# usnistgov/optbayesexpt

Hardware: AMD Instinct MI355X
Metric: model-evals/sec (settings x particles) per opt_setting+update cycle, fp64 (higher is better)
Workload: dtype f64; 1 GPU; c3: Lorentzian 3-param, 65 536 settings x 1 048 576 particles; n_settings=65536, n_particles=1048576, settings_per_rank=65536

## Files before the change

include/obe_hip.h:

```cpp
#ifndef OBE_HIP_H
#define OBE_HIP_H

#include <stdint.h>

#ifdef __cplusplus
extern "C" {
#endif

#define OBE_API __attribute__((visibility("default")))

#define OBE_ABI_VERSION 3
#define OBE_MAX_CONSTS 8
#define OBE_MAX_CHANNELS 8
#define OBE_MAX_SETDIMS 8
#define OBE_MAX_DIMS 32
#define OBE_FAST_DIMS 16
#define OBE_CLOUD_MAX_DIMS 1024

enum obe_model_id {
    OBE_MODEL_LORENTZ = 1,
    OBE_MODEL_LINE_AB = 2,
    OBE_MODEL_LINE_MB = 3,
    OBE_MODEL_FIRST_PARAM = 4,
    OBE_MODEL_RABI = 5,
// ... 173 lines not shown
                        void* d_ws, int64_t ws_bytes, void* stream);

#define OBE_WS_RESULT_OFFSET 2
#define OBE_WS_RESULT_TAIL(d_ws, ws_bytes) ((double*)((char*)(d_ws) + ((ws_bytes) & ~(int64_t)7) - 48))
#define OBE_NOISE_FROM_MOMENTS(r0, r1, r2, r3) \
    (-(int64_t)1 - ((int64_t)(r0) | ((int64_t)(r1) << 5) | ((int64_t)(r2) << 10) | ((int64_t)(r3) << 15)))
#define OBE_SWEEP_SHIFTED 1
#define OBE_SWEEP_SAFE 2
#define OBE_SWEEP_SPECULATIVE 8
#define OBE_SWEEP_NOWAIT 16
#define OBE_SWEEP_CELLS 4
#define OBE_CELL_RHO_INV 4
#define OBE_CELL_ORDER 28
#define OBE_CELL_MAX 128
#define OBE_CELL_MIN_GAIN 2
OBE_API int obe_sweep_cells_plan(double x_min, double x_max, double d, int64_t n_settings, int64_t n_draws);
#define OBE_SWEEP_BINS 32
#define OBE_BIN_MAX 128
OBE_API int obe_sweep_bins_plan(double x_min, double x_max, double d, int64_t n_settings, int64_t n_draws);
OBE_API int obe_sweep_bins_eval_waves(int64_t n_settings);
OBE_API int obe_sweep_settings_per_lane(int64_t n_settings);
OBE_API int obe_sweep_settings_per_lane_for(int64_t n_settings, int64_t n_draws);
OBE_API int obe_sweep_utility(const obe_model* m,
                      const double* d_settings, int64_t ld_s, int64_t n_settings,
                      const double* d_particles, int64_t ld_p, int64_t n_particles,
                      const double* d_weights, const int64_t* d_draw_idx, int64_t n_draws,
                      const double* d_moments, int32_t shifted,
                      const double* d_noise_var, int64_t noise_ld,
                      const double* d_cost, double cost_scalar,
                      double* d_yvar, double* d_utility,
                      double* h_best, int64_t* h_best_idx, double* h_kappa,
                      void* d_ws, int64_t ws_bytes, void* stream);
OBE_API int64_t obe_sweep_bins_keep_bytes(int64_t n_draws);
#define OBE_SWEEP_BINS_KEPT 64
OBE_API int obe_sweep_utility_keep(const obe_model* m,
                      const double* d_settings, int64_t ld_s, int64_t n_settings,
                      const double* d_particles, int64_t ld_p, int64_t n_particles,
                      const double* d_weights, const int64_t* d_draw_idx, int64_t n_draws,
                      const double* d_moments, int32_t shifted,
                      const double* d_noise_var, int64_t noise_ld,
                      const double* d_cost, double cost_scalar,
                      double* d_yvar, double* d_utility,
                      double* h_value, int64_t* h_index, double* h_factor,
                      void* d_ws, int64_t ws_bytes, void* stream,
                      void* d_keep, int64_t keep_bytes);

OBE_API int obe_yspace_variance(const double* d_yspace, int64_t n_draws, int32_t n_channels,
                        int64_t n_settings, double* d_yvar, void* stream);
OBE_API int obe_utility_argmax(const double* d_yvar, int32_t n_channels, int64_t n_settings,
                       const double* d_noise_var, int64_t noise_ld,
                       const double* d_cost, double cost_scalar,
                       double* d_utility, double* h_best, int64_t* h_best_idx,
                       void* d_ws, int64_t ws_bytes, void* stream);
OBE_API int obe_argmax(const double* d_v, int64_t n, double* h_best, int64_t* h_best_idx,
               void* d_ws, int64_t ws_bytes, void* stream);

OBE_API int obe_eval_draws(const obe_model* m, const double* d_settings, int64_t ld_s, int64_t n_settings,
                   const double* d_particles, int64_t ld_p, int64_t n_particles,
                   const int64_t* d_draw_idx, int64_t n_draws, double* d_yspace, void* stream);
OBE_API int obe_yspace_add_noise(double* d_yspace, int64_t n_draws, int32_t n_channels, int64_t n_settings,
                         const double* d_noise, void* stream);
OBE_API int obe_yspace_maxmin(const double* d_yspace, int64_t n_draws, int64_t n_columns, double* d_span2, void* stream);
OBE_API int obe_yspace_entropy(const double* d_yspace, int64_t n_draws, int64_t n_columns, int32_t as_variance,
                       double* d_scratch, double* d_out, void* stream);
OBE_API int obe_kld_utility(const double* d_entropy_y, int32_t n_channels, int64_t n_settings,
                    const double* d_entropy_noise, double* d_utility, void* stream);
// ... 127 lines not shown
```

optbayesexpt_amd/_lib.py:

```python
import ctypes
import os
import re

import numpy as np

HERE = os.path.dirname(os.path.abspath(__file__))
LIB_PATH = os.path.join(HERE, "lib", "libobe_hip.so")
HEADER_PATH = os.path.join(os.path.dirname(HERE), "include", "obe_hip.h")



def _header_constants(path=HEADER_PATH):
    text = open(path).read()
    return {k: int(v) for k, v in re.findall(r"^#define\s+(OBE_[A-Z_]+)\s+(-?\d+)\s*(?:/\*.*)?$", text, flags=re.M)}


_H = _header_constants()
OBE_ABI_VERSION = _H["OBE_ABI_VERSION"]
OBE_MAX_CONSTS = _H["OBE_MAX_CONSTS"]
OBE_MAX_CHANNELS = _H["OBE_MAX_CHANNELS"]
OBE_MAX_SETDIMS = _H["OBE_MAX_SETDIMS"]
OBE_MAX_DIMS = _H["OBE_MAX_DIMS"]
OBE_FAST_DIMS = _H["OBE_FAST_DIMS"]
OBE_CLOUD_MAX_DIMS = _H["OBE_CLOUD_MAX_DIMS"]
# ... 53 lines not shown
def _ctype(c_type):
    m = re.fullmatch(r"(?:const\s+)?(\w+)\s*(\**)", c_type)
    if m and m[2]:
        return _POINTERS.get(m[1] + m[2], c_void_p)
    if m and m[1] in _SCALARS:
        return _SCALARS[m[1]]
    raise TypeError(f"no ctypes binding for the C type {c_type!r} of include/obe_hip.h")


def _prototypes(header_path=HEADER_PATH):
    text = re.sub(r"/\*.*?\*/", "", open(header_path).read(), flags=re.S)
    protos = {}
    for ret, name, params in re.findall(r"^OBE_API\s+([^(]+?)\s*\b(obe_\w+)\s*\(([^)]*)\)\s*;", text, flags=re.M):
        args = []
        for param in [] if params.strip() == "void" else params.split(","):
            m = re.fullmatch(r"(.+?)\s*\b(\w+)", param.strip())
            if m is None:
                raise TypeError(f"{name}: cannot read the parameter {param.strip()!r} of include/obe_hip.h")
            args.append((_ctype(m[1]), m[2]))
        protos[name] = (_ctype(ret), args)
    return protos


PROTOTYPES = _prototypes()


MODEL_ENTRY_POINTS = ("obe_model_validate", "obe_workspace_bytes", "obe_sweep_settings_per_lane",
                      "obe_sweep_settings_per_lane_for", "obe_bayes_update_model",
                      "obe_bayes_update_model_moments", "obe_bayes_update_model_moments_enqueue",
                      "obe_strict_sums",
                      "obe_bayes_update_sweep",
                      "obe_eval_over_particles",
                      "obe_eval_over_settings", "obe_sweep_utility", "obe_sweep_kernel_time", "obe_sweep_timing",
                      "obe_sweep_utility_keep", "obe_sweep_bins_keep_bytes",
                      "obe_eval_draws",
                      "obe_predictive_workspace_bytes", "obe_predictive_moments", "obe_predictive_quantiles",
                      "obe_predictive_score_workspace_bytes", "obe_predictive_logpdf", "obe_predictive_tails",
                      "obe_predictive_reading_workspace_bytes", "obe_predictive_reading_quantiles",
                      "obe_output_covariance_workspace_bytes", "obe_output_covariance",
                      "obe_records_loglik_workspace_bytes", "obe_records_loglik",
                      "obe_output_cross_covariance_workspace_bytes", "obe_output_cross_covariance",
                      "obe_signal_noise_likelihood", "obe_signal_noise_workspace_bytes", "obe_signal_noise_variance")


class HipLib:

    def __init__(self, path=LIB_PATH, plugin=False, allow_variant=False):
        if not os.path.exists(path):
            raise ImportError(
                f"{path} not found: the HIP library has not been built.  Run "
                "`python -m optbayesexpt_amd.build` (needs hipcc).  optbayesexpt_amd has "
                "no CPU fallback.")
        import torch
        self.path = path
        self.cdll = ctypes.CDLL(path, mode=ctypes.RTLD_LOCAL if plugin else ctypes.RTLD_GLOBAL)
        names = MODEL_ENTRY_POINTS + ("obe_abi_version", "obe_last_error", "obe_source_fingerprint") if plugin \
            else tuple(PROTOTYPES)
        for name in names:
            restype, params = PROTOTYPES[name]
            fn = getattr(self.cdll, name)
            fn.restype = restype
            fn.argtypes = [ctype for ctype, _ in params]
        abi = self.cdll.obe_abi_version()
        if abi != OBE_ABI_VERSION:
            raise ImportError(f"libobe_hip ABI {abi} does not match this package ({OBE_ABI_VERSION})")
        from . import build
        built_from = self.cdll.obe_source_fingerprint().decode()
# ... 170 lines not shown
```

optbayesexpt_amd/csrc/obe_sweep.hip:

```cpp
#include <cstdlib>

#include "obe_update.h"
#include "obe_sweep_common.h"
#include "obe_sweep_cells.h"
#include "obe_sweep_bins.h"

namespace obe {

constexpr int kMaxChunks = 1024;
constexpr int kFinMaxBlocks = 65536;

static int64_t argmax_slots(int64_t n_settings) {
    return std::max<int64_t>(kMaxBlocks, (n_settings + kFinSettings - 1) / kFinSettings);
}

static SweepPlan plan_sweep(int64_t ns, int64_t nd, int cost = 1, int max_spt = 8) {
    SweepPlan p;
    p.spt = ns >= 4096 || (ns >= 2048 && nd >= 131072) ? 8 : (ns >= 1024 ? 4 : (ns >= 512 ? 2 : 1));
    if (p.spt > max_spt) p.spt = max_spt;
    p.tiles_x = static_cast<int>((ns + (int64_t)kWave * p.spt - 1) / ((int64_t)kWave * p.spt));
    const int64_t by_work = static_cast<int64_t>((double)ns * (double)nd * (double)cost / 1.25e6);
    const int64_t target_blocks = std::max<int64_t>(1536, std::min<int64_t>(4608, by_work));
    int64_t want = (target_blocks + p.tiles_x - 1) / p.tiles_x;
    if (want > 8) want = (want + 7) / 8 * 8;
// ... 665 lines not shown
    double replaced = (double)n_settings * (double)n_draws * kDirectSlots;
    if (cells == 3) {
        const double ncells = std::floor((x_max / d - x_min / d) * (1.0 / LorentzCells::kWidth)) + 1.0;
        replaced = (double)n_draws * std::ceil(ncells / kWave) * kWave * kCellSlots;
    }
    const double bins = (double)n_settings * OBE_BIN_MAX * kBinEvalSlots + (double)n_draws * kBinDrawSlots + kBinFixedSlots;
    return replaced >= OBE_CELL_MIN_GAIN * bins ? 3 : 1;
}

int obe_sweep_bins_eval_waves(int64_t n_settings) { return plan_bin_eval_waves(n_settings < 1 ? 1 : n_settings); }

int obe_sweep_settings_per_lane_for(int64_t n_settings, int64_t n_draws) {
    if (n_settings < 1) n_settings = 1;
    if (n_draws < 1) return obe_sweep_settings_per_lane(n_settings);
    if (one_workgroup_sweep(n_settings, n_draws)) return 1;
    return plan_sweep(n_settings, n_draws).spt;
}

int64_t obe_workspace_bytes(int64_t n_particles, int64_t n_settings, int32_t n_channels, int32_t n_dims) {
    if (n_particles < 1) n_particles = 1;
    if (n_settings < 1) n_settings = 1;
    if (n_channels < 1) n_channels = 1;
    if (n_dims < 1) n_dims = 1;
    const int packed_w = max_packed_width(n_dims);
    int64_t b = sweep_ws_bytes_bound(n_settings, n_particles, n_channels, packed_w);
    b = std::max(b, moments_ws_bytes(n_dims));
    b = std::max(b, update_ws_bytes(n_dims));
    b = std::max(b, scan_ws_bytes(n_particles));
    b = std::max(b, resample_wide_ws_bytes(n_dims));
    return b + 64 * (int64_t)sizeof(double);
}

int64_t obe_sweep_bins_keep_bytes(int64_t n_draws) { return BinKeepLayout::bytes(n_draws < 1 ? 1 : n_draws); }

int obe_sweep_utility(const obe_model* m, const double* d_settings, int64_t ld_s, int64_t n_settings,
                      const double* d_particles, int64_t ld_p, int64_t n_particles, const double* d_weights,
                      const int64_t* d_draw_idx, int64_t n_draws, const double* d_moments, int32_t shifted,
                      const double* d_noise_var, int64_t noise_ld, const double* d_cost, double cost_scalar,
                      double* d_yvar, double* d_utility, double* h_best, int64_t* h_best_idx, double* h_kappa,
                      void* d_ws, int64_t ws_bytes, void* stream) {
    return obe_sweep_utility_keep(m, d_settings, ld_s, n_settings, d_particles, ld_p, n_particles, d_weights, d_draw_idx,
                                  n_draws, d_moments, shifted, d_noise_var, noise_ld, d_cost, cost_scalar, d_yvar, d_utility,
                                  h_best, h_best_idx, h_kappa, d_ws, ws_bytes, stream, nullptr, 0);
}

int obe_sweep_utility_keep(const obe_model* m, const double* d_settings, int64_t ld_s, int64_t n_settings,
                           const double* d_particles, int64_t ld_p, int64_t n_particles, const double* d_weights,
                           const int64_t* d_draw_idx, int64_t n_draws, const double* d_moments, int32_t shifted,
                           const double* d_noise_var, int64_t noise_ld, const double* d_cost, double cost_scalar,
                           double* d_yvar, double* d_utility, double* h_best, int64_t* h_best_idx, double* h_kappa,
                           void* d_ws, int64_t ws_bytes, void* stream, void* d_keep, int64_t keep_bytes) {
    if (!d_noise_var || !d_yvar || !d_utility) return bad_arg("obe_sweep_utility: bad output/noise pointer");
    if (d_keep && reinterpret_cast<uintptr_t>(d_keep) % 16) return bad_arg("obe_sweep_utility_keep: d_keep is not 16-byte aligned");
    SweepCall c;
    if (int rc = prepare_sweep(SweepInputs{m, d_settings, ld_s, n_settings, d_particles, ld_p, n_particles, d_weights,
                                           d_draw_idx, n_draws, d_moments, shifted, d_ws, ws_bytes, d_keep, keep_bytes}, c))
        return rc;
    const obe_model& mm = c.mm;
    SweepPlan& plan = c.plan;
    SweepArgs& a = c.a;
    const SweepWs& w = c.w;
    hipStream_t st = as_stream(stream);
    UtilArgs ua;
    if (int rc = make_util_args(ua, d_noise_var, noise_ld, d_cost, cost_scalar, mm.n_channels, mm.n_params)) return rc;
    const bool speculative = shifted & OBE_SWEEP_SPECULATIVE;
    const bool nowait = speculative || (shifted & OBE_SWEEP_NOWAIT);
// ... 202 lines not shown
```

optbayesexpt_amd/csrc/obe_sweep_bins.h:

```cpp
#pragma once
#include "obe_sweep_common.h"

namespace obe {

struct BinPlan {
    double origin;
    int nbins;
    unsigned poison;
};
constexpr int kBinMinmaxBlocks = 256;
constexpr int kBinMaxUnits = 2048;
constexpr int kBinChunk = 1024;
constexpr int kBinFoldGroups = 16;
constexpr int kBinScanPer = kBinMaxUnits / kBlock;
constexpr double kBinEvalSlots = 8.0 * LorentzBins::kOrder + 16.0;
constexpr double kBinDrawSlots = 4.0 * LorentzBins::kOrder + 8.0;
constexpr double kBinFixedSlots = 80.0 * 3.9e7;

struct BinUnits {
    int nunits;
    int64_t per;
};
static BinUnits plan_bin_units(int64_t nd) {
    BinUnits u;
// ... 2 lines not shown
    u.nunits = static_cast<int>((nd + u.per - 1) / u.per);
    return u;
}
struct BinEvalShape {
    int waves, groups;
};
constexpr BinEvalShape kBinEvalShapes[] = {{8, 1}, {6, 2}, {3, 4}};
constexpr int kBinEvalWavesPerCU = 12, kChipCUs = 256;
static int plan_bin_eval_waves(int64_t ns) {
    const int64_t groups = (ns + kWave - 1) / kWave;
    for (const BinEvalShape& f : kBinEvalShapes)
        if (groups <= (int64_t)kChipCUs * f.groups * (kBinEvalWavesPerCU / (f.groups * f.waves))) return f.waves;
    return 1;
}
static int64_t bin_max_items(int64_t nd) { return (nd + kBinChunk - 1) / kBinChunk + LorentzBins::kMaxBins; }
struct BinLayout {
    static constexpr int64_t kPlan = 0, kRan = 3, kStarts = 4;
    static constexpr int64_t kMinmax = kStarts + 132;
    static constexpr int64_t kTotals = kMinmax + 3 * kBinMinmaxBlocks;
    static constexpr int64_t kCounts = kTotals + LorentzBins::kMaxBins / 2;
    static constexpr int64_t kCoef = kCounts + (int64_t)LorentzBins::kMaxBins * kBinMaxUnits / 2;
    static constexpr int64_t kPart = kCoef + (int64_t)LorentzBins::kMaxBins * LorentzBins::kRow;
    static int64_t sorted(int64_t nd) { return kPart + bin_max_items(nd) * LorentzBins::kRow; }
    static int64_t doubles(int64_t nd) { return sorted(nd) + 4 * nd; }
};
static_assert(BinLayout::kPart % 2 == 0 && LorentzBins::kRow % 2 == 0, "the sorted records are 16-byte aligned");

struct BinKeep {
    BinPlan plan;
    unsigned mark;
    int nd;
    unsigned long long dbits;
    unsigned mismatch;
    unsigned pad[7];
};
static_assert(sizeof(BinKeep) == 64, "the head of the keep buffer is 16 ints");
constexpr unsigned kBinKeepMark = 0x6b455042u;
struct BinKeepLayout {
    static constexpr int64_t kStarts = sizeof(BinKeep) / sizeof(int);
    static constexpr int64_t kDest = (kStarts + 2 * (LorentzBins::kMaxBins + 2) + 3) & ~(int64_t)3;
    static int64_t bytes(int64_t nd) { return ((kDest + nd) * (int64_t)sizeof(int) + 15) & ~(int64_t)15; }
};

#ifndef OBE_PLUGIN_MODEL_HEADER
struct BinSweepPtrs {
    BinPlan* plan;
    unsigned* ran;
    int* binstart;
    int* itemstart;
    BinKeep* keep;
    int* dest;
    int* code;
    int reuse;
    int keep_nd;
    unsigned long long keep_dbits;
    unsigned call;
    double* minmax;
    int* totals;
    int* counts;
    double* coef;
    double* part;
    double* sorted;
};

__device__ __forceinline__ bool bin_keep_refused(const BinSweepPtrs& q) {
    if (!q.reuse) return false;
    const BinKeep* k = q.keep;
    return !(k->mark == kBinKeepMark && k->nd == q.keep_nd && k->dbits == q.keep_dbits);
}

__device__ __forceinline__ double bin_tau0(const SweepArgs& a, int64_t p) {
    double w;
    const int64_t src = draw_source(a, p, w);
    return a.particles[src] / a.m.consts[0];
}

__device__ __forceinline__ void bin_record(const SweepArgs& a, int64_t p, double2& ra, double2& rb) {
    using M = Lorentz<1>;
    static_assert(packed_width<M>() == 4 && M::NPK == 3, "the sorted records are 32 bytes");
    double w, pk[4];
    const int64_t src = draw_source(a, p, w);
    const double sw = sqrt(w);
    M::pack(ParamRef{a.particles + src, a.ld_p}, a.moments + 2, a.m, sw, pk);
    ra = double2{pk[0], pk[1]};
    rb = double2{pk[2], sw};
}

constexpr int kBinRankBits = 24;
static_assert((((int64_t)1 << 30) + kBinMaxUnits - 1) / kBinMaxUnits <= ((int64_t)1 << kBinRankBits)
                  && LorentzBins::kMaxBins <= (1 << (31 - kBinRankBits)),
              "a unit of a cloud of 2^30 draws (BinForm::selected) has at most 2^19 draws: rank and bin share an int");
__device__ __forceinline__ int bin_code(int bin, int rank) { return (bin << kBinRankBits) | rank; }

__global__ __launch_bounds__(kBlock) void bin_minmax_kernel(SweepArgs a, BinSweepPtrs q) {
    constexpr int NW = kBlock / kWave;
    __shared__ double slo[NW], shi[NW];
    __shared__ int sbad[NW];
    if (sweep_aborted(a.abort)) return;
    if (q.keep && blockIdx.x == 0 && threadIdx.x == 0) q.keep->mark = 0u;
    double* __restrict__ minmax = q.minmax;
    double lo = INFINITY, hi = -INFINITY;
    int bad = 0;
    for (int64_t p = (int64_t)blockIdx.x * kBlock + threadIdx.x; p < a.nd; p += (int64_t)gridDim.x * kBlock) {
        const double t = bin_tau0(a, p);
        bad |= !(fabs(t) <= kDblMax);
        lo = fmin(lo, t);
        hi = fmax(hi, t);
    }
#pragma unroll
    for (int o = kWave / 2; o > 0; o >>= 1) {
        lo = fmin(lo, __shfl_down(lo, o, kWave));
        hi = fmax(hi, __shfl_down(hi, o, kWave));
        bad |= __shfl_down(bad, o, kWave);
    }
    if ((threadIdx.x & (kWave - 1)) == 0) {
        slo[threadIdx.x / kWave] = lo;
        shi[threadIdx.x / kWave] = hi;
        sbad[threadIdx.x / kWave] = bad;
    }
    __syncthreads();
    if (threadIdx.x != 0) return;
    for (int g = 1; g < NW; ++g) {
        lo = fmin(lo, slo[g]);
        hi = fmax(hi, shi[g]);
        bad |= sbad[g];
    }
    minmax[blockIdx.x] = lo;
    minmax[kBinMinmaxBlocks + blockIdx.x] = hi;
    minmax[2 * kBinMinmaxBlocks + blockIdx.x] = bad ? 1.0 : 0.0;
}

__device__ __forceinline__ BinPlan bin_plan_of(const SweepArgs& a, const double* __restrict__ minmax, int nblocks) {
// ... 3 lines not shown
#pragma unroll
    for (int g = 0; g < kBinMinmaxBlocks / kWave; ++g) {
        const int b = g * kWave + lane;
        const bool have = b < nblocks;
        lo = fmin(lo, have ? minmax[b] : INFINITY);
        hi = fmax(hi, have ? minmax[kBinMinmaxBlocks + b] : -INFINITY);
        bad |= have ? minmax[2 * kBinMinmaxBlocks + b] != 0.0 : 0;
    }
#pragma unroll
    for (int o = kWave / 2; o > 0; o >>= 1) {
        lo = fmin(lo, __shfl_xor(lo, o, kWave));
        hi = fmax(hi, __shfl_xor(hi, o, kWave));
        bad |= __shfl_xor(bad, o, kWave);
    }
    const double d = a.m.consts[0];
    const double n = floor((hi - lo) * (1.0 / LorentzBins::kWidth)) + 1.0;
    const bool ok = !bad && d > 0.0 && d <= kDblMax && fabs(lo) <= kDblMax && fabs(hi) <= kDblMax
                    && n <= (double)LorentzBins::kMaxBins;
    return BinPlan{lo, ok ? static_cast<int>(n) : 0, ok ? 0u : 1u};
}

__device__ __forceinline__ int wave_exclusive(int v, int& total) {
    const int lane = threadIdx.x & (kWave - 1);
    int inc = v;
#pragma unroll
    for (int o = 1; o < kWave; o <<= 1) {
        const int up = __shfl_up(inc, o, kWave);
        inc += lane >= o ? up : 0;
    }
    total = __shfl(inc, kWave - 1, kWave);
    return inc - v;
}

template <bool SCATTER>
__global__ __launch_bounds__(kBlock) void bin_group_kernel(SweepArgs a, int64_t per, int nunits, int mm_blocks,
                                                           BinSweepPtrs q) {
    using LB = LorentzBins;
    if (sweep_aborted(a.abort)) return;
    const int lane = threadIdx.x & (kWave - 1);
    const int unit = blockIdx.x * (kBlock / kWave) + threadIdx.x / kWave;
    BinPlan plan;
    if constexpr (SCATTER) {
        plan = *q.plan;
        if (q.keep && blockIdx.x == 0 && threadIdx.x == 0) {
            q.keep->nd = static_cast<int>(a.nd);
            q.keep->dbits = q.keep_dbits;
            q.keep->mismatch = 0u;
            q.keep->mark = kBinKeepMark;
        }
    } else {
        plan = bin_plan_of(a, q.minmax, mm_blocks);
        if (blockIdx.x == 0 && threadIdx.x == 0) *q.plan = plan;
    }
    const int nbins = __builtin_amdgcn_readfirstlane(plan.nbins);
    if (nbins == 0) return;
    int c0 = 0, c1 = 0;
    if constexpr (SCATTER) {
        const int t0 = q.totals[lane], t1 = q.totals[lane + kWave];
        int sum0, sum1, isum0, isum1;
        const int e0 = wave_exclusive(t0, sum0), e1 = sum0 + wave_exclusive(t1, sum1);
        const int i0 = wave_exclusive((t0 + kBinChunk - 1) / kBinChunk, isum0);
        const int i1 = isum0 + wave_exclusive((t1 + kBinChunk - 1) / kBinChunk, isum1);
        if (unit == 0) {
            q.binstart[lane] = e0;
            q.binstart[lane + kWave] = e1;
            q.itemstart[lane] = i0;
            q.itemstart[lane + kWave] = i1;
            if (lane == 0) {
                q.binstart[LB::kMaxBins] = sum0 + sum1;
                q.itemstart[LB::kMaxBins] = isum0 + isum1;
            }
        }
        if (unit >= nunits) return;
        c0 = e0 + q.counts[lane * kBinMaxUnits + unit];
        c1 = e1 + q.counts[(lane + kWave) * kBinMaxUnits + unit];
    }
    if (unit >= nunits) return;
    const int64_t begin = (int64_t)unit * per;
    const int64_t end = begin + per < a.nd ? begin + per : a.nd;
    for (int64_t i0 = begin; i0 < end; i0 += kWave) {
        const int64_t i = i0 + lane;
        const bool live = i < end;
        if constexpr (SCATTER) {
            const int code = live ? q.code[i] : 0;
            const int bin = code >> kBinRankBits;
            const int first0 = __shfl(c0, bin & (kWave - 1), kWave), first1 = __shfl(c1, bin & (kWave - 1), kWave);
            const int pos = (bin < kWave ? first0 : first1) + (code & ((1 << kBinRankBits) - 1));
            if (live && pos >= 0 && pos < a.nd) {
                double2 ra, rb;
                bin_record(a, i, ra, rb);
                double2* __restrict__ out = reinterpret_cast<double2*>(q.sorted) + 2 * (int64_t)pos;
                out[0] = ra;
                out[1] = rb;
            }
            if (q.dest && live) q.dest[i] = pos;
        } else {
            const int bin = live ? LB::bin_of(plan.origin, bin_tau0(a, i), nbins) : -1;
            int rank = 0;
            unsigned long long todo = __ballot(live);
            while (todo) {
                const int b = __builtin_amdgcn_readlane(bin, __builtin_ctzll(todo));
                const unsigned long long same = __ballot(bin == b);
                const int figure = __builtin_amdgcn_readlane(b < kWave ? c0 : c1, b & (kWave - 1));
                if (bin == b) rank = figure + __popcll(same & ((1ull << lane) - 1ull));
                const int n = __popcll(same);
                if (lane == (b & (kWave - 1))) {
                    if (b < kWave) c0 += n;
                    else c1 += n;
                }
                todo &= ~same;
            }
            if (live) q.code[i] = bin_code(bin, rank);
        }
    }
    if constexpr (!SCATTER) {
        q.counts[lane * kBinMaxUnits + unit] = c0;
        q.counts[(lane + kWave) * kBinMaxUnits + unit] = c1;
    }
}

__global__ __launch_bounds__(kBlock) void bin_scatter_pack_kernel(SweepArgs a, BinSweepPtrs q) {
    using LB = LorentzBins;
    if (sweep_aborted(a.abort)) return;
    if (bin_keep_refused(q)) return;
    const int nbins = __builtin_amdgcn_readfirstlane(q.plan->nbins);
    if (nbins <= 0 || nbins > LB::kMaxBins) return;
    const double origin = q.plan->origin;
    for (int64_t p = (int64_t)blockIdx.x * kBlock + threadIdx.x; p < a.nd; p += (int64_t)gridDim.x * kBlock) {
        double2 ra, rb;
        bin_record(a, p, ra, rb);
        const int pos = q.dest[p];
        const double t = (ra.x - origin) * (1.0 / LB::kWidth);
        bool ok = t >= 0.0 && t < (double)nbins && pos >= 0 && pos < a.nd;
        if (ok) {
            const int b = LB::bin_of(origin, ra.x, nbins);
            ok = q.binstart[b] <= pos && pos < q.binstart[b + 1];
        }
        if (ok) {
            double2* __restrict__ out = reinterpret_cast<double2*>(q.sorted) + 2 * (int64_t)pos;
            out[0] = ra;
            out[1] = rb;
        } else {
            q.keep->mismatch = q.call;
        }
    }
}

__global__ __launch_bounds__(kBlock) void bin_scan_kernel(int nunits, BinSweepPtrs q, const unsigned* abort) {
    __shared__ int wsum[kBlock / kWave];
    if (sweep_aborted(abort)) return;
    const int nbins = __builtin_amdgcn_readfirstlane(q.plan->nbins);
    const int bin = blockIdx.x;
    if (nbins == 0) return;
    if (bin >= nbins) {
        if (threadIdx.x == 0) q.totals[bin] = 0;
        return;
    }
    int* __restrict__ row = q.counts + bin * kBinMaxUnits;
    int v[kBinScanPer], mine = 0;
#pragma unroll
    for (int u = 0; u < kBinScanPer; ++u) {
        const int k = threadIdx.x * kBinScanPer + u;
        v[u] = k < nunits ? row[k] : 0;
        mine += v[u];
    }
    int wtotal;
    int before = wave_exclusive(mine, wtotal);
    if ((threadIdx.x & (kWave - 1)) == 0) wsum[threadIdx.x / kWave] = wtotal;
    __syncthreads();
    int total = 0;
#pragma unroll
    for (int g = 0; g < kBlock / kWave; ++g) {
        if (g < (int)threadIdx.x / kWave) before += wsum[g];
        total += wsum[g];
    }
#pragma unroll
    for (int u = 0; u < kBinScanPer; ++u) {
// ... 9 lines not shown
    constexpr int H = (N + 1) / 2;
    const bool upper = (lane & DIST) != 0;
    double k[H];
#pragma unroll
    for (int i = 0; i < H; ++i) {
        const double lo = v[i], hi = H + i < N ? v[H + i] : 0.0;
        const double mine = upper ? hi : lo, send = upper ? lo : hi;
        k[i] = mine + __shfl_xor(send, DIST, kWave);
    }
    if constexpr (DIST > 1) {
        halving_reduce<H, DIST / 2>(k, lane, out);
    } else {
        static_assert(H == 2, "64 lanes x 2 values: at most 128 sums");
        out[0] = k[0];
        out[1] = k[1];
    }
}
template <int N>
__device__ __forceinline__ int halving_index(int lane, int e) {
    int n[7];
    n[0] = N;
#pragma unroll
    for (int l = 0; l < 6; ++l) n[l + 1] = (n[l] + 1) / 2;
    int j = e;
    bool real = true;
#pragma unroll
    for (int l = 5; l >= 0; --l) {
        j += ((lane >> (5 - l)) & 1) * n[l + 1];
        real = real && j < n[l];
    }
    return real ? j : -1;
}

__global__ __launch_bounds__(kWave) void bin_moments_kernel(BinSweepPtrs q, const unsigned* abort) {
    using LB = LorentzBins;
    if (sweep_aborted(abort)) return;
    if (bin_keep_refused(q)) return;
    const int nbins = __builtin_amdgcn_readfirstlane(q.plan->nbins);
    if (nbins == 0) return;
    const int lane = threadIdx.x, item = blockIdx.x;
    if (item >= q.itemstart[LB::kMaxBins]) return;
    const int s0 = q.itemstart[lane], s1 = q.itemstart[lane + kWave];
    const int bin = __popcll(__ballot(lane < nbins && s0 <= item)) + __popcll(__ballot(lane + kWave < nbins && s1 <= item)) - 1;
    const int first = q.binstart[bin] + (item - q.itemstart[bin]) * kBinChunk;
    const int last = q.binstart[bin + 1];
    const int end = first + kBinChunk < last ? first + kBinChunk : last;
    const double tb = LB::centre(q.plan->origin, bin);
    const double2* __restrict__ rec = reinterpret_cast<const double2*>(q.sorted);
    LB::Sums z;
    z.clear();
    int i = first + lane;
    double2 ra = double2{0.0, 0.0}, rb = ra;
    if (i < end) {
        ra = rec[2 * (int64_t)i];
        rb = rec[2 * (int64_t)i + 1];
    }
    while (i < end) {
        const int in = i + kWave;
        double2 na = ra, nb = rb;
        if (in < end) {
            na = rec[2 * (int64_t)in];
            nb = rec[2 * (int64_t)in + 1];
        }
        const double pk[4] = {ra.x, ra.y, rb.x, rb.y};
        LB::add_draw(tb, pk, z);
        ra = na;
        rb = nb;
        i = in;
    }
    double v[LB::kCoefs], kept[2];
#pragma unroll
    for (int k = 0; k < LB::kOrder; ++k) {
        v[k] = z.M1[k];
        v[LB::kOrder + k] = z.M2[k];
        v[2 * LB::kOrder + k] = z.M3[k];
    }
    v[3 * LB::kOrder] = z.c1;
    v[3 * LB::kOrder + 1] = z.c2;
    halving_reduce<LB::kCoefs, kWave / 2>(v, lane, kept);
    double* __restrict__ out = q.part + (int64_t)item * LB::kRow;
#pragma unroll
    for (int e = 0; e < 2; ++e) {
        const int j = halving_index<LB::kCoefs>(lane, e);
        if (j < 0) continue;
        const bool m3 = j >= 2 * LB::kOrder && j < 3 * LB::kOrder;
        out[j] = kept[e] * (m3 ? (double)(j - 2 * LB::kOrder + 1) : 1.0);
    }
}

__global__ __launch_bounds__(kBinFoldGroups * kWave) void bin_fold_kernel(BinSweepPtrs q, const unsigned* abort) {
    using LB = LorentzBins;
    __shared__ double acc[kBinFoldGroups][kWave];
    if (sweep_aborted(abort)) return;
    if (bin_keep_refused(q)) return;
    const int nbins = __builtin_amdgcn_readfirstlane(q.plan->nbins);
    const int bin = blockIdx.x >> 1, co = (blockIdx.x & 1) * kWave + (threadIdx.x & (kWave - 1));
    if (bin >= nbins) return;
    const int first = __builtin_amdgcn_readfirstlane(q.itemstart[bin]);
    const int n = __builtin_amdgcn_readfirstlane(q.itemstart[bin + 1]) - first;
    if (n == 0) return;
    const bool live = co < LB::kCoefs;
// ... 122 lines not shown
        S2 = a2 + C2;
    }
    if (blockIdx.x == 0 && threadIdx.x == 0) *q.ran = seq;
    if (W > 1 && wid != 0) return;
    if (!f.yvar) {
        if (s >= a.ns) return;
        a.part1[s] = S1;
        a.part2[s] = S2;
        a.cs_out[s] = 0.0;
        return;
    }
    const int64_t group = (int64_t)blockIdx.x * G + grp;
    if (group * kWave >= a.ns) return;
    double kappa = 0.0;
    Best best{-INFINITY, INT64_MAX};
    if (s < a.ns) {
        const double var = variance_of_moments(0.0 + S1, 0.0 + S2, f.full_mode ? a.moments[0] : 1.0, 0.0, kappa);
        f.yvar[s] = var;
        const double u = utility_of(&var, 1, 1, s, f.ua);
        f.utility[s] = u;
        best = Best{u, s};
    }
    wave_best(best, kappa);
    if (lane == 0) {
        f.bv[group] = best.v;
        f.bi[group] = best.i;
        f.bk[group] = kappa;
    }
}

struct BinForm {
    bool on = false;
    BinSweepPtrs q{};

    static bool selected(const obe_model& m, int flags, int64_t ns, const int64_t* d_draw_idx, int64_t n_draws,
                         int64_t nd) {
        return (flags & OBE_SWEEP_BINS) && nd <= ((int64_t)1 << 30) && expansion_applies(m, flags, ns, d_draw_idx, n_draws);
    }
    void carve(double* base, double* packed, int64_t nd, const obe_model& m, int flags, const int64_t* d_draw_idx,
               void* d_keep, int64_t keep_bytes) {
        using BL = BinLayout;
        q.plan = reinterpret_cast<BinPlan*>(base + BL::kPlan);
        q.ran = reinterpret_cast<unsigned*>(base + BL::kRan);
        q.binstart = reinterpret_cast<int*>(base + BL::kStarts);
        q.itemstart = q.binstart + LorentzBins::kMaxBins + 2;
        q.minmax = base + BL::kMinmax;
        q.totals = reinterpret_cast<int*>(base + BL::kTotals);
        q.counts = reinterpret_cast<int*>(base + BL::kCounts);
        q.coef = base + BL::kCoef;
        q.part = base + BL::kPart;
        q.sorted = base + BL::sorted(nd);
        q.code = reinterpret_cast<int*>(packed);
        if (d_keep && !d_draw_idx && keep_bytes >= BinKeepLayout::bytes(nd)) {
            static std::atomic<unsigned> calls{0};
            int* ints = static_cast<int*>(d_keep);
            q.keep = static_cast<BinKeep*>(d_keep);
            q.plan = &q.keep->plan;
            q.binstart = ints + BinKeepLayout::kStarts;
            q.itemstart = q.binstart + LorentzBins::kMaxBins + 2;
            q.dest = ints + BinKeepLayout::kDest;
            q.code = q.dest;
            q.reuse = (flags & OBE_SWEEP_BINS_KEPT) != 0;
            q.keep_nd = static_cast<int>(nd);
            memcpy(&q.keep_dbits, &m.consts[0], sizeof q.keep_dbits);
            q.call = ++calls;
            if (q.call == 0u) q.call = ++calls;
        }
    }
    int before(const SweepArgs& a, hipStream_t st) const {
        if (!q.reuse) return 0;
        bin_scatter_pack_kernel<<<stream_blocks(a.nd, kBlock), kBlock, 0, st>>>(a, q);
        OBE_CHECK_LAUNCH("bin_scatter_pack_kernel");
        return 0;
    }
    int sweep(SweepPlan& p, const SweepArgs& a, unsigned seq, const BinFinish& f, hipStream_t st) const {
        using LB = LorentzBins;
        if (!q.reuse) {
            const BinUnits units = plan_bin_units(a.nd);
            const int mm_blocks = static_cast<int>(std::min<int64_t>(kBinMinmaxBlocks, (a.nd + kBlock - 1) / kBlock));
            bin_minmax_kernel<<<mm_blocks, kBlock, 0, st>>>(a, q);
            OBE_CHECK_LAUNCH("bin_minmax_kernel");
            const unsigned group_blocks = (unsigned)((units.nunits + kBlock / kWave - 1) / (kBlock / kWave));
            bin_group_kernel<false><<<group_blocks, kBlock, 0, st>>>(a, units.per, units.nunits, mm_blocks, q);
            OBE_CHECK_LAUNCH("bin_group_kernel<count>");
            bin_scan_kernel<<<LB::kMaxBins, kBlock, 0, st>>>(units.nunits, q, a.abort);
            OBE_CHECK_LAUNCH("bin_scan_kernel");
            bin_group_kernel<true><<<group_blocks, kBlock, 0, st>>>(a, units.per, units.nunits, mm_blocks, q);
            OBE_CHECK_LAUNCH("bin_group_kernel<scatter>");
        }
        bin_moments_kernel<<<(unsigned)bin_max_items(a.nd), kWave, 0, st>>>(q, a.abort);
        OBE_CHECK_LAUNCH("bin_moments_kernel");
        bin_fold_kernel<<<2 * LB::kMaxBins, kBinFoldGroups * kWave, 0, st>>>(q, a.abort);
        OBE_CHECK_LAUNCH("bin_fold_kernel");
        p.nchunks = 1;
        const unsigned groups = (unsigned)((a.ns + kWave - 1) / kWave);
        switch (plan_bin_eval_waves(a.ns)) {
            case 8: bin_eval_kernel<1, 8><<<groups, 8 * kWave, 0, st>>>(a, q, seq, f); break;
            case 6: bin_eval_kernel<2, 6><<<(groups + 1) / 2, 12 * kWave, 0, st>>>(a, q, seq, f); break;
            case 3: bin_eval_kernel<4, 3><<<(groups + 3) / 4, 12 * kWave, 0, st>>>(a, q, seq, f); break;
            default: bin_eval_kernel<4, 1><<<(groups + 3) / 4, kBlock, 0, st>>>(a, q, seq, f);
        }
        OBE_CHECK_LAUNCH("bin_eval_kernel");
        return 0;
    }
};
#endif

}
```

optbayesexpt_amd/obe_base.py:

```python
import os
import warnings

import numpy as np
import torch

from . import _batch, _bounds, _design, _devrng, _drift, _interest, _lib, _predictive, _reading, _scoring
from ._sweepstate import Attempt, Form, Pending, SweepState, Ticket
from . import models as _models
from ._mirror import Mirror, TrackedArray
from .models import DeviceModel
from .particlepdf import ParticlePDF, _P, _ptr

DEFAULT_N_DRAWS = 30
MAX_ENTROPY_DRAWS = 2048
rng = np.random.default_rng()

UTILITY_METHODS = ["variance_approx", "pseudo_utility", "full_kld_utility", "max_min",
                   "variance_full", "parameter_variance"]
SELECTION_METHODS = ["optimal", "good", "random"]


_OVERRIDDEN = {}


# ... 826 lines not shown
            return None
        key = (self._s_begin, self._s_end, self.n_particles)
        cells, bins = self._cells_plan, self._bins_plan
        if cells is None or cells[0] != key:
            x, n = self.allsettings[0, self._s_begin:self._s_end], self._s_end - self._s_begin
            with np.errstate(all="ignore"):
                lo, hi = float(np.min(x)), float(np.max(x))
            cells = self._cells_plan = (key, int(self._mlib.cdll.obe_sweep_cells_plan(
                lo, hi, float(self.cons[0]), n, self.n_particles)))
            if self._shard is not None:
                x, n = self.allsettings[0], -(-self._n_settings // self._shard.world_size)
                with np.errstate(all="ignore"):
                    lo, hi = float(np.min(x)), float(np.max(x))
            bins = self._bins_plan = (key, int(self._mlib.cdll.obe_sweep_bins_plan(
                lo, hi, float(self.cons[0]), n, self.n_particles)))
        return cells[1], bins[1], self._bins_keep_key()

    def _cell_form_wanted(self):
        forms = self._expansion_forms()
        return forms is not None and self._sweeps.cells_wanted(self.tuning_parameters, forms[0])

    def _bin_form_wanted(self):
        forms = self._expansion_forms()
        return forms is not None and self._sweeps.bins_wanted(self.tuning_parameters, forms[1], forms[2][0])

    def _bins_keep_key(self):
        return (self._particles.version, float(self.cons[0]), self.n_particles)

    def _bins_kept(self):
        return self._sweeps.bins_kept(self._bins_keep_key())

    def _bins_keep_buffer(self):
        keep = self.__dict__.get("_bins_keep")
        if keep is None or keep[0] != self.n_particles:
            nbytes = int(self._mlib.cdll.obe_sweep_bins_keep_bytes(self.n_particles))
            keep = self._bins_keep = (self.n_particles,
                                      torch.zeros((nbytes + 3) // 4, dtype=torch.int32, device=self._device))
            self._sweeps.keep_buffer_replaced()
        return keep[1]

    def _settings_per_lane(self, n_draws=0):
        cache = self.__dict__.setdefault("_spt_local", {})
        spt = cache.get(n_draws)
        if spt is None:
            lengths = {max(self._s_end - self._s_begin, 1)}
            if self._shard is not None:
                base, extra = divmod(self._n_settings, self._shard.world_size)
                lengths = {max(base, 1), base + 1} if extra else {max(base, 1)}
            spt = cache[n_draws] = max(int(self._mlib.cdll.obe_sweep_settings_per_lane_for(n, n_draws))
                                       for n in lengths)
        return spt

    def _sweep_needs_range_check(self, n_draws=0):
        dm = self._device_model
        return bool(dm is not None and dm.safe_sweep and self._settings_per_lane(n_draws) >= dm.safe_sweep_min_spt)

    def _apply_range_hint(self):
        hint = getattr(self._device_model, "range_hint", None)
        pm = self._particles
        state = self._sweeps
        sharded = self._shard is not None
        if hint is None or not pm._host_valid or state.range_hint_key == pm.version:
            return
        if sharded and not pm.host_born:
            return
        state.range_hint_key = pm.version
        n_local = self._s_end - self._s_begin
        if n_local <= 0 and not sharded:
            return
# ... 223 lines not shown
```

Measured before the change: 604100 billion model-evals/s.

## Keep sorted raw particle records so reuse refresh only rewrites sqrt weights

Enlarges the bins keep buffer to hold sorted per-particle records (tau0, amplitude, offset) plus a separate sqrt-weight array. When the grouping is reused, a new refresh kernel only rewrites sqrt(w) at each kept destination instead of re-gathering and repacking every particle, and the moments kernel rebuilds the packed values from the records and the current mean offset. The counting pass also replaces the per-wave ballot loop with a bitwise bin-match ballot and prefetches eight particle loads ahead. The cost is a larger keep buffer, extra reads in the moments kernel, and the assumption that particle positions are unchanged whenever the record mark is set.

```diff
diff --git a/include/obe_hip.h b/include/obe_hip.h
--- a/include/obe_hip.h
+++ b/include/obe_hip.h
@@ -229,6 +229,7 @@
                       double* h_best, int64_t* h_best_idx, double* h_kappa,
                       void* d_ws, int64_t ws_bytes, void* stream);
 OBE_API int64_t obe_sweep_bins_keep_bytes(int64_t n_draws);
+OBE_API int64_t obe_sweep_bins_keep_records_bytes(int64_t n_draws);
 #define OBE_SWEEP_BINS_KEPT 64
 OBE_API int obe_sweep_utility_keep(const obe_model* m,
                       const double* d_settings, int64_t ld_s, int64_t n_settings,
diff --git a/optbayesexpt_amd/_lib.py b/optbayesexpt_amd/_lib.py
--- a/optbayesexpt_amd/_lib.py
+++ b/optbayesexpt_amd/_lib.py
@@ -109,7 +109,7 @@
                       "obe_bayes_update_sweep",
                       "obe_eval_over_particles",
                       "obe_eval_over_settings", "obe_sweep_utility", "obe_sweep_kernel_time", "obe_sweep_timing",
-                      "obe_sweep_utility_keep", "obe_sweep_bins_keep_bytes",
+                      "obe_sweep_utility_keep", "obe_sweep_bins_keep_bytes", "obe_sweep_bins_keep_records_bytes",
                       "obe_eval_draws",
                       "obe_predictive_workspace_bytes", "obe_predictive_moments", "obe_predictive_quantiles",
                       "obe_predictive_score_workspace_bytes", "obe_predictive_logpdf", "obe_predictive_tails",
diff --git a/optbayesexpt_amd/csrc/obe_sweep.hip b/optbayesexpt_amd/csrc/obe_sweep.hip
--- a/optbayesexpt_amd/csrc/obe_sweep.hip
+++ b/optbayesexpt_amd/csrc/obe_sweep.hip
@@ -721,6 +721,9 @@
 }
 
 int64_t obe_sweep_bins_keep_bytes(int64_t n_draws) { return BinKeepLayout::bytes(n_draws < 1 ? 1 : n_draws); }
+int64_t obe_sweep_bins_keep_records_bytes(int64_t n_draws) {
+    return BinKeepLayout::records_bytes(n_draws < 1 ? 1 : n_draws);
+}
 
 int obe_sweep_utility(const obe_model* m, const double* d_settings, int64_t ld_s, int64_t n_settings,
                       const double* d_particles, int64_t ld_p, int64_t n_particles, const double* d_weights,
diff --git a/optbayesexpt_amd/csrc/obe_sweep_bins.h b/optbayesexpt_amd/csrc/obe_sweep_bins.h
--- a/optbayesexpt_amd/csrc/obe_sweep_bins.h
+++ b/optbayesexpt_amd/csrc/obe_sweep_bins.h
@@ -58,7 +58,8 @@
     int nd;
     unsigned long long dbits;
     unsigned mismatch;
-    unsigned pad[7];
+    unsigned records;
+    unsigned pad[6];
 };
 static_assert(sizeof(BinKeep) == 64, "the head of the keep buffer is 16 ints");
 constexpr unsigned kBinKeepMark = 0x6b455042u;
@@ -66,6 +67,10 @@
     static constexpr int64_t kStarts = sizeof(BinKeep) / sizeof(int);
     static constexpr int64_t kDest = (kStarts + 2 * (LorentzBins::kMaxBins + 2) + 3) & ~(int64_t)3;
     static int64_t bytes(int64_t nd) { return ((kDest + nd) * (int64_t)sizeof(int) + 15) & ~(int64_t)15; }
+    static constexpr int64_t kRecord = 3;
+    static int64_t records_at(int64_t nd) { return bytes(nd); }
+    static int64_t sw_at(int64_t nd) { return records_at(nd) + ((kRecord * 8 * nd + 15) & ~(int64_t)15); }
+    static int64_t records_bytes(int64_t nd) { return sw_at(nd) + ((8 * nd + 15) & ~(int64_t)15); }
 };
 
 #ifndef OBE_PLUGIN_MODEL_HEADER
@@ -89,27 +94,57 @@
     double* sorted;
 };
 
+struct BinRecords {
+    double* rec;
+    double* sw;
+    const double* bbar;
+};
+
 __device__ __forceinline__ bool bin_keep_refused(const BinSweepPtrs& q) {
     if (!q.reuse) return false;
     const BinKeep* k = q.keep;
     return !(k->mark == kBinKeepMark && k->nd == q.keep_nd && k->dbits == q.keep_dbits);
 }
 
-__device__ __forceinline__ double bin_tau0(const SweepArgs& a, int64_t p) {
+__device__ __forceinline__ double bin_x0(const SweepArgs& a, int64_t p) {
     double w;
     const int64_t src = draw_source(a, p, w);
-    return a.particles[src] / a.m.consts[0];
-}
-
-__device__ __forceinline__ void bin_record(const SweepArgs& a, int64_t p, double2& ra, double2& rb) {
+    return a.particles[src];
+}
+__device__ __forceinline__ double bin_tau0(const SweepArgs& a, int64_t p) { return bin_x0(a, p) / a.m.consts[0]; }
+
+__device__ __forceinline__ void bin_pk(double tau0, double amp, double b, double bbar, double sw, double (&pk)[4]) {
+    pk[0] = tau0;
+    pk[1] = sw * amp;
+    pk[2] = sw * (b - bbar);
+    pk[3] = sw;
+}
+__device__ __forceinline__ void bin_particle(const SweepArgs& a, int64_t p, double (&part)[3], double& sw) {
     using M = Lorentz<1>;
     static_assert(packed_width<M>() == 4 && M::NPK == 3, "the sorted records are 32 bytes");
-    double w, pk[4];
+    double w;
     const int64_t src = draw_source(a, p, w);
-    const double sw = sqrt(w);
-    M::pack(ParamRef{a.particles + src, a.ld_p}, a.moments + 2, a.m, sw, pk);
+    sw = sqrt(w);
+    part[0] = a.particles[src] / a.m.consts[0];
+    part[1] = a.particles[src + a.ld_p];
+    part[2] = a.particles[src + 2 * a.ld_p];
+}
+__device__ __forceinline__ void bin_record(const SweepArgs& a, int64_t p, double2& ra, double2& rb) {
+    double part[3], sw, pk[4];
+    bin_particle(a, p, part, sw);
+    bin_pk(part[0], part[1], part[2], a.moments[4], sw, pk);
     ra = double2{pk[0], pk[1]};
-    rb = double2{pk[2], sw};
+    rb = double2{pk[2], pk[3]};
+}
+
+__device__ __forceinline__ void bin_store_particle(const SweepArgs& a, int64_t p, int pos, const BinRecords& r) {
+    double part[3], sw;
+    bin_particle(a, p, part, sw);
+    double* __restrict__ out = r.rec + BinKeepLayout::kRecord * (int64_t)pos;
+    out[0] = part[0];
+    out[1] = part[1];
+    out[2] = part[2];
+    r.sw[pos] = sw;
 }
 
 constexpr int kBinRankBits = 24;
@@ -117,13 +152,19 @@
                   && LorentzBins::kMaxBins <= (1 << (31 - kBinRankBits)),
               "a unit of a cloud of 2^30 draws (BinForm::selected) has at most 2^19 draws: rank and bin share an int");
 __device__ __forceinline__ int bin_code(int bin, int rank) { return (bin << kBinRankBits) | rank; }
+constexpr int kBinIndexBits = 7;
+constexpr int kBinGroupAhead = 8;
+static_assert(LorentzBins::kMaxBins == 1 << kBinIndexBits, "a bin index is matched bit by bit (bin_group_kernel<false>)");
 
 __global__ __launch_bounds__(kBlock) void bin_minmax_kernel(SweepArgs a, BinSweepPtrs q) {
     constexpr int NW = kBlock / kWave;
     __shared__ double slo[NW], shi[NW];
     __shared__ int sbad[NW];
     if (sweep_aborted(a.abort)) return;
-    if (q.keep && blockIdx.x == 0 && threadIdx.x == 0) q.keep->mark = 0u;
+    if (q.keep && blockIdx.x == 0 && threadIdx.x == 0) {
+        q.keep->mark = 0u;
+        q.keep->records = 0u;
+    }
     double* __restrict__ minmax = q.minmax;
     double lo = INFINITY, hi = -INFINITY;
     int bad = 0;
@@ -193,10 +234,11 @@
     return inc - v;
 }
 
-template <bool SCATTER>
+template <bool SCATTER, bool RECORDS = false>
 __global__ __launch_bounds__(kBlock) void bin_group_kernel(SweepArgs a, int64_t per, int nunits, int mm_blocks,
-                                                           BinSweepPtrs q) {
+                                                           BinSweepPtrs q, BinRecords r) {
     using LB = LorentzBins;
+    static_assert(SCATTER || !RECORDS, "the counting pass stores no record");
     if (sweep_aborted(a.abort)) return;
     const int lane = threadIdx.x & (kWave - 1);
     const int unit = blockIdx.x * (kBlock / kWave) + threadIdx.x / kWave;
@@ -208,6 +250,7 @@
             q.keep->dbits = q.keep_dbits;
             q.keep->mismatch = 0u;
             q.keep->mark = kBinKeepMark;
+            if constexpr (RECORDS) q.keep->records = kBinKeepMark;
         }
     } else {
         plan = bin_plan_of(a, q.minmax, mm_blocks);
@@ -239,47 +282,93 @@
     if (unit >= nunits) return;
     const int64_t begin = (int64_t)unit * per;
     const int64_t end = begin + per < a.nd ? begin + per : a.nd;
-    for (int64_t i0 = begin; i0 < end; i0 += kWave) {
-        const int64_t i = i0 + lane;
-        const bool live = i < end;
-        if constexpr (SCATTER) {
+    if constexpr (SCATTER) {
+        for (int64_t i0 = begin; i0 < end; i0 += kWave) {
+            const int64_t i = i0 + lane;
+            const bool live = i < end;
             const int code = live ? q.code[i] : 0;
             const int bin = code >> kBinRankBits;
             const int first0 = __shfl(c0, bin & (kWave - 1), kWave), first1 = __shfl(c1, bin & (kWave - 1), kWave);
             const int pos = (bin < kWave ? first0 : first1) + (code & ((1 << kBinRankBits) - 1));
             if (live && pos >= 0 && pos < a.nd) {
-                double2 ra, rb;
-                bin_record(a, i, ra, rb);
-                double2* __restrict__ out = reinterpret_cast<double2*>(q.sorted) + 2 * (int64_t)pos;
-                out[0] = ra;
-                out[1] = rb;
+                if constexpr (RECORDS) {
+                    bin_store_particle(a, i, pos, r);
+                } else {
+                    double2 ra, rb;
+                    bin_record(a, i, ra, rb);
+                    double2* __restrict__ out = reinterpret_cast<double2*>(q.sorted) + 2 * (int64_t)pos;
+                    out[0] = ra;
+                    out[1] = rb;
+                }
             }
             if (q.dest && live) q.dest[i] = pos;
+        }
+    } else {
+        __shared__ int tally[kBlock / kWave][LB::kMaxBins];
+        int* count = tally[threadIdx.x / kWave];
+        count[lane] = 0;
+        count[lane + kWave] = 0;
+        __builtin_amdgcn_fence(__ATOMIC_SEQ_CST, "wavefront");
+        const double d = a.m.consts[0];
+        const unsigned long long below = (1ull << lane) - 1ull;
+        auto trip = [&](int64_t i0, double x0) {
+            const int64_t i = i0 + lane;
+            const bool live = i < end;
+            const int bin = live ? LB::bin_of(plan.origin, x0 / d, nbins) : -1;
+            unsigned long long same = __ballot(live);
+#pragma unroll
+            for (int k = 0; k < kBinIndexBits; ++k) {
+                const bool bit = (bin >> k) & 1;
+                const unsigned long long have = __ballot(bit);
+                same &= bit ? have : ~have;
+            }
+            if (!live) same = 0ull;
+            const int sofar = live ? count[bin] : 0;
+            if (live && (same & below) == 0ull) count[bin] = sofar + __popcll(same);
+            __builtin_amdgcn_fence(__ATOMIC_SEQ_CST, "wavefront");
+            if (live) q.code[i] = bin_code(bin, sofar + __popcll(same & below));
+        };
+        for (int64_t i0 = begin; i0 < end; i0 += kBinGroupAhead * kWave) {
+            double x0[kBinGroupAhead];
+#pragma unroll
+            for (int k = 0; k < kBinGroupAhead; ++k) {
+                const int64_t i = i0 + k * kWave + lane;
+                x0[k] = bin_x0(a, i < end ? i : end - 1);
+            }
+#pragma unroll
+            for (int k = 0; k < kBinGroupAhead; ++k)
+                if (i0 + k * kWave < end) trip(i0 + k * kWave, x0[k]);
+        }
+        q.counts[lane * kBinMaxUnits + unit] = count[lane];
+        q.counts[(lane + kWave) * kBinMaxUnits + unit] = count[lane + kWave];
+    }
+}
+
+template <bool RECORDS>
+__device__ __forceinline__ void bin_scatter_pack_draw(const SweepArgs& a, const BinSweepPtrs& q, const BinRecords& r,
+                                                      double origin, int nbins, int64_t p) {
+    using LB = LorentzBins;
+    double2 ra, rb;
+    bin_record(a, p, ra, rb);
+    const int pos = q.dest[p];
+    const double t = (ra.x - origin) * (1.0 / LB::kWidth);
+    bool ok = t >= 0.0 && t < (double)nbins && pos >= 0 && pos < a.nd;
+    if (ok) {
+        const int b = LB::bin_of(origin, ra.x, nbins);
+        ok = q.binstart[b] <= pos && pos < q.binstart[b + 1];
+    }
+    if (ok) {
+        if constexpr (RECORDS) {
+            bin_store_particle(a, p, pos, r);
         } else {
-            const int bin = live ? LB::bin_of(plan.origin, bin_tau0(a, i), nbins) : -1;
-            int rank = 0;
-            unsigned long long todo = __ballot(live);
-            while (todo) {
-                const int b = __builtin_amdgcn_readlane(bin, __builtin_ctzll(todo));
-                const unsigned long long same = __ballot(bin == b);
-                const int figure = __builtin_amdgcn_readlane(b < kWave ? c0 : c1, b & (kWave - 1));
-                if (bin == b) rank = figure + __popcll(same & ((1ull << lane) - 1ull));
-                const int n = __popcll(same);
-                if (lane == (b & (kWave - 1))) {
-                    if (b < kWave) c0 += n;
-                    else c1 += n;
-                }
-                todo &= ~same;
-            }
-            if (live) q.code[i] = bin_code(bin, rank);
-        }
-    }
-    if constexpr (!SCATTER) {
-        q.counts[lane * kBinMaxUnits + unit] = c0;
-        q.counts[(lane + kWave) * kBinMaxUnits + unit] = c1;
-    }
-}
-
+            double2* __restrict__ out = reinterpret_cast<double2*>(q.sorted) + 2 * (int64_t)pos;
+            out[0] = ra;
+            out[1] = rb;
+        }
+    } else {
+        q.keep->mismatch = q.call;
+    }
+}
 __global__ __launch_bounds__(kBlock) void bin_scatter_pack_kernel(SweepArgs a, BinSweepPtrs q) {
     using LB = LorentzBins;
     if (sweep_aborted(a.abort)) return;
@@ -287,23 +376,28 @@
     const int nbins = __builtin_amdgcn_readfirstlane(q.plan->nbins);
     if (nbins <= 0 || nbins > LB::kMaxBins) return;
     const double origin = q.plan->origin;
-    for (int64_t p = (int64_t)blockIdx.x * kBlock + threadIdx.x; p < a.nd; p += (int64_t)gridDim.x * kBlock) {
-        double2 ra, rb;
-        bin_record(a, p, ra, rb);
-        const int pos = q.dest[p];
-        const double t = (ra.x - origin) * (1.0 / LB::kWidth);
-        bool ok = t >= 0.0 && t < (double)nbins && pos >= 0 && pos < a.nd;
-        if (ok) {
-            const int b = LB::bin_of(origin, ra.x, nbins);
-            ok = q.binstart[b] <= pos && pos < q.binstart[b + 1];
-        }
-        if (ok) {
-            double2* __restrict__ out = reinterpret_cast<double2*>(q.sorted) + 2 * (int64_t)pos;
-            out[0] = ra;
-            out[1] = rb;
-        } else {
-            q.keep->mismatch = q.call;
-        }
+    for (int64_t p = (int64_t)blockIdx.x * kBlock + threadIdx.x; p < a.nd; p += (int64_t)gridDim.x * kBlock)
+        bin_scatter_pack_draw<false>(a, q, BinRecords{}, origin, nbins, p);
+}
+
+__global__ __launch_bounds__(kBlock) void bin_refresh_kernel(SweepArgs a, BinSweepPtrs q, BinRecords r, int64_t per) {
+    using LB = LorentzBins;
+    if (sweep_aborted(a.abort)) return;
+    if (bin_keep_refused(q)) return;
+    const int nbins = __builtin_amdgcn_readfirstlane(q.plan->nbins);
+    if (nbins <= 0 || nbins > LB::kMaxBins) return;
+    const int64_t begin = (int64_t)blockIdx.x * per;
+    const int64_t end = begin + per < a.nd ? begin + per : a.nd;
+    if (q.keep->records == kBinKeepMark) {
+        const double* __restrict__ w = a.weights;
+        const int* __restrict__ dest = q.dest;
+        for (int64_t p = begin + threadIdx.x; p < end; p += kBlock) {
+            const int pos = dest[p];
+            if (pos >= 0 && pos < a.nd) r.sw[pos] = sqrt(w[p]);
+        }
+    } else {
+        const double origin = q.plan->origin;
+        for (int64_t p = begin + threadIdx.x; p < end; p += kBlock) bin_scatter_pack_draw<true>(a, q, r, origin, nbins, p);
     }
 }
 
@@ -379,7 +473,8 @@
     return real ? j : -1;
 }
 
-__global__ __launch_bounds__(kWave) void bin_moments_kernel(BinSweepPtrs q, const unsigned* abort) {
+template <bool RECORDS>
+__global__ __launch_bounds__(kWave) void bin_moments_kernel(BinSweepPtrs q, const unsigned* abort, BinRecords r) {
     using LB = LorentzBins;
     if (sweep_aborted(abort)) return;
     if (bin_keep_refused(q)) return;
@@ -393,27 +488,60 @@
     const int last = q.binstart[bin + 1];
     const int end = first + kBinChunk < last ? first + kBinChunk : last;
     const double tb = LB::centre(q.plan->origin, bin);
-    const double2* __restrict__ rec = reinterpret_cast<const double2*>(q.sorted);
     LB::Sums z;
     z.clear();
-    int i = first + lane;
-    double2 ra = double2{0.0, 0.0}, rb = ra;
-    if (i < end) {
-        ra = rec[2 * (int64_t)i];
-        rb = rec[2 * (int64_t)i + 1];
-    }
-    while (i < end) {
-        const int in = i + kWave;
-        double2 na = ra, nb = rb;
-        if (in < end) {
-            na = rec[2 * (int64_t)in];
-            nb = rec[2 * (int64_t)in + 1];
-        }
-        const double pk[4] = {ra.x, ra.y, rb.x, rb.y};
-        LB::add_draw(tb, pk, z);
-        ra = na;
-        rb = nb;
-        i = in;
+    if constexpr (!RECORDS) {
+        const double2* __restrict__ rec = reinterpret_cast<const double2*>(q.sorted);
+        int i = first + lane;
+        double2 ra = double2{0.0, 0.0}, rb = ra;
+        if (i < end) {
+            ra = rec[2 * (int64_t)i];
+            rb = rec[2 * (int64_t)i + 1];
+        }
+        while (i < end) {
+            const int in = i + kWave;
+            double2 na = ra, nb = rb;
+            if (in < end) {
+                na = rec[2 * (int64_t)in];
+                nb = rec[2 * (int64_t)in + 1];
+            }
+            const double pk[4] = {ra.x, ra.y, rb.x, rb.y};
+            LB::add_draw(tb, pk, z);
+            ra = na;
+            rb = nb;
+            i = in;
+        }
+    } else {
+        const double bbar = *r.bbar;
+        const double* __restrict__ rec = r.rec;
+        const double* __restrict__ rsw = r.sw;
+        constexpr int64_t R = BinKeepLayout::kRecord;
+        int i = first + lane;
+        double tau0 = 0.0, amp = 0.0, b = 0.0, sw = 0.0;
+        if (i < end) {
+            tau0 = rec[R * i];
+            amp = rec[R * i + 1];
+            b = rec[R * i + 2];
+            sw = rsw[i];
+        }
+        while (i < end) {
+            const int in = i + kWave;
+            double ntau0 = tau0, namp = amp, nb = b, nsw = sw;
+            if (in < end) {
+                ntau0 = rec[R * in];
+                namp = rec[R * in + 1];
+                nb = rec[R * in + 2];
+                nsw = rsw[in];
+            }
+            double pk[4];
+            bin_pk(tau0, amp, b, bbar, sw, pk);
+            LB::add_draw(tb, pk, z);
+            tau0 = ntau0;
+            amp = namp;
+            b = nb;
+            sw = nsw;
+            i = in;
+        }
     }
     double v[LB::kCoefs], kept[2];
 #pragma unroll
@@ -602,6 +730,7 @@
 struct BinForm {
     bool on = false;
     BinSweepPtrs q{};
+    BinRecords r{};
 
     static bool selected(const obe_model& m, int flags, int64_t ns, const int64_t* d_draw_idx, int64_t n_draws,
                          int64_t nd) {
@@ -635,10 +764,21 @@
             memcpy(&q.keep_dbits, &m.consts[0], sizeof q.keep_dbits);
             q.call = ++calls;
             if (q.call == 0u) q.call = ++calls;
+            if (keep_bytes >= BinKeepLayout::records_bytes(nd)) {
+                char* bytes = static_cast<char*>(d_keep);
+                r.rec = reinterpret_cast<double*>(bytes + BinKeepLayout::records_at(nd));
+                r.sw = reinterpret_cast<double*>(bytes + BinKeepLayout::sw_at(nd));
+            }
         }
     }
     int before(const SweepArgs& a, hipStream_t st) const {
         if (!q.reuse) return 0;
+        if (r.rec) {
+            const int64_t per = plan_bin_units(a.nd).per * (kBlock / kWave);
+            bin_refresh_kernel<<<(unsigned)((a.nd + per - 1) / per), kBlock, 0, st>>>(a, q, r, per);
+            OBE_CHECK_LAUNCH("bin_refresh_kernel");
+            return 0;
+        }
         bin_scatter_pack_kernel<<<stream_blocks(a.nd, kBlock), kBlock, 0, st>>>(a, q);
         OBE_CHECK_LAUNCH("bin_scatter_pack_kernel");
         return 0;
@@ -651,14 +791,23 @@
             bin_minmax_kernel<<<mm_blocks, kBlock, 0, st>>>(a, q);
             OBE_CHECK_LAUNCH("bin_minmax_kernel");
             const unsigned group_blocks = (unsigned)((units.nunits + kBlock / kWave - 1) / (kBlock / kWave));
-            bin_group_kernel<false><<<group_blocks, kBlock, 0, st>>>(a, units.per, units.nunits, mm_blocks, q);
+            bin_group_kernel<false><<<group_blocks, kBlock, 0, st>>>(a, units.per, units.nunits, mm_blocks, q, r);
             OBE_CHECK_LAUNCH("bin_group_kernel<count>");
             bin_scan_kernel<<<LB::kMaxBins, kBlock, 0, st>>>(units.nunits, q, a.abort);
             OBE_CHECK_LAUNCH("bin_scan_kernel");
-            bin_group_kernel<true><<<group_blocks, kBlock, 0, st>>>(a, units.per, units.nunits, mm_blocks, q);
+            if (r.rec)
+                bin_group_kernel<true, true><<<group_blocks, kBlock, 0, st>>>(a, units.per, units.nunits, mm_blocks, q, r);
+            else
+                bin_group_kernel<true><<<group_blocks, kBlock, 0, st>>>(a, units.per, units.nunits, mm_blocks, q, r);
             OBE_CHECK_LAUNCH("bin_group_kernel<scatter>");
         }
-        bin_moments_kernel<<<(unsigned)bin_max_items(a.nd), kWave, 0, st>>>(q, a.abort);
+        if (r.rec) {
+            BinRecords rr = r;
+            rr.bbar = a.moments + 4;
+            bin_moments_kernel<true><<<(unsigned)bin_max_items(a.nd), kWave, 0, st>>>(q, a.abort, rr);
+        } else {
+            bin_moments_kernel<false><<<(unsigned)bin_max_items(a.nd), kWave, 0, st>>>(q, a.abort, r);
+        }
         OBE_CHECK_LAUNCH("bin_moments_kernel");
         bin_fold_kernel<<<2 * LB::kMaxBins, kBinFoldGroups * kWave, 0, st>>>(q, a.abort);
         OBE_CHECK_LAUNCH("bin_fold_kernel");
diff --git a/optbayesexpt_amd/obe_base.py b/optbayesexpt_amd/obe_base.py
--- a/optbayesexpt_amd/obe_base.py
+++ b/optbayesexpt_amd/obe_base.py
@@ -882,9 +882,11 @@
 
     def _bins_keep_buffer(self):
         keep = self.__dict__.get("_bins_keep")
-        if keep is None or keep[0] != self.n_particles:
-            nbytes = int(self._mlib.cdll.obe_sweep_bins_keep_bytes(self.n_particles))
-            keep = self._bins_keep = (self.n_particles,
+        size = ("obe_sweep_bins_keep_bytes" if self.tuning_parameters.get("sweep_bins_keep", True) == "grouping"
+                else "obe_sweep_bins_keep_records_bytes")
+        if keep is None or keep[0] != (self.n_particles, size):
+            nbytes = int(getattr(self._mlib.cdll, size)(self.n_particles))
+            keep = self._bins_keep = ((self.n_particles, size),
                                       torch.zeros((nbytes + 3) // 4, dtype=torch.int32, device=self._device))
             self._sweeps.keep_buffer_replaced()
         return keep[1]
```

Result: faster. 633400 billion model-evals/s, median of 6 (+4.8%).
